# liruiluo/VLA-Adapter

Hardware: AMD Instinct MI355X
Metric: fine-tune samples/sec (224px img + 32-tok prompt), adapter-only, fwd+bwd+AdamW (higher is better)
Workload: dtype bf16

## Files before the change

vla_adapter_amd/csrc/gemm256.hip:

```cpp
#include <type_traits>
#include "gemm_epilogue.h"
#include "gemm_params.h"

namespace {

constexpr int BK = 64;
constexpr int HT = 16384;
constexpr int LDS_BYTES = 8 * HT;
constexpr int STG = 8192;

#define VLA_MMA_QUADRANT(Q, FB, FA)                                                                                                   \
  do {                                                                                                                                \
    if constexpr (F8) {                                                                                                               \
      _Pragma("unroll") for (int ni = 0; ni < 2; ++ni)                                                                                \
        _Pragma("unroll") for (int mi = 0; mi < 4; ++mi)                                                                              \
          Q[ni][mi] = __builtin_amdgcn_mfma_scale_f32_16x16x128_f8f6f4(cat8(FB[ni][0], FB[ni][1]), cat8(FA[mi][0], FA[mi][1]), Q[ni][mi], \
                                                                       0, 0, 0, 0x7f7f7f7f, 0, 0x7f7f7f7f);                            \
    } else {                                                                                                                          \
      _Pragma("unroll") for (int s = 0; s < 2; ++s)                                                                                   \
        _Pragma("unroll") for (int ni = 0; ni < 2; ++ni)                                                                              \
          _Pragma("unroll") for (int mi = 0; mi < 4; ++mi)                                                                            \
            Q[ni][mi] = __builtin_amdgcn_mfma_f32_16x16x32_bf16(FB[ni][s], FA[mi][s], Q[ni][mi], 0, 0, 0);                            \
    }                                                                                                                                 \
  } while (0)

template <int EPI, bool F8 = false, bool RES = true, bool R2 = false, bool EXT = false>
__global__ __launch_bounds__(512) void gemm256_kernel(GemmP p) {
  extern __shared__ __attribute__((aligned(16))) char smem[];
  constexpr int EB = F8 ? 1 : 2;
  constexpr bool HAS_RES = EPI == 0 && RES;
  constexpr bool PRE = EPI != 2;
  const int tid = threadIdx.x, lane = tid & 63;
  const int wid = __builtin_amdgcn_readfirstlane(tid >> 6);
  const int wr = wid >> 2, wc = wid & 3;

  const int G = gridDim.x, bid = blockIdx.x;
  const int total = p.ntiles * p.batch;
  const int q8 = total >> 3, r8 = total & 7;
  const int xcd = bid & 7;
  auto rstart = [&](int x) { return x < r8 ? x * (q8 + 1) : r8 * (q8 + 1) + (x - r8) * q8; };
  int vt = bid;
  constexpr int GM = 6;
  int m0, n0, z;
  const char* Ab; const char* Bb;
  unsigned oa[2][2], ob[2][2];
  unsigned oa2[EXT ? 2 : 1][2], ob2[EXT ? 2 : 1][2];
  auto setup = [&](int swz) {
    int sl = lane;
    asm volatile("" : "+v"(sl));
    const int kc = ((sl & 7) ^ ((sl >> 3) & 7)) * 16;
    const int lrow = sl >> 3;
    int gA = p.gA;
    asm volatile("" : "+s"(gA));
    int ntl = p.ntiles;
    asm volatile("" : "+s"(ntl));
    z = swz / ntl;
    const int tl = swz - z * ntl;
    int br = ntl / p.tiles_n, bc = p.tiles_n;
    asm volatile("" : "+s"(br), "+s"(bc));
    const int pgb = GM * bc;
    const int grp = tl / pgb, rem = tl - grp * pgb;
    const int gmr = min(GM, br - grp * GM);
    m0 = (grp * GM + rem % gmr) * 256;
    n0 = (rem / gmr) * 256;
    Ab = reinterpret_cast<const char*>(p.A) + (long long)z * p.sA * EB;
    Bb = reinterpret_cast<const char*>(p.B) + (long long)z * p.sB * EB;
#pragma unroll
    for (int h = 0; h < 2; ++h)
#pragma unroll
      for (int j = 0; j < 2; ++j) {
        const int ra = min(m0 + wr * 128 + h * 64 + (wid & 3) * 16 + j * 8 + lrow, p.M - 1);
        oa[h][j] = (unsigned)(grouped_row(ra, gA, p.sgA, p.lda) * EB + kc);
        const int rb = min(n0 + (wid >> 1) * 64 + h * 32 + (wid & 1) * 16 + j * 8 + lrow, p.N - 1);
        ob[h][j] = (unsigned)((long long)rb * p.ldb * EB + kc);
        if constexpr (EXT) {
          oa2[h][j] = (unsigned)((long long)ra * p.lda2 * 2 + kc);
          ob2[h][j] = (unsigned)((long long)rb * p.ldb2 * 2 + kc);
        }
      }
  };
  const unsigned wdst = (unsigned)(size_t)((__attribute__((address_space(3))) char*)smem) + wid * 2048;
  auto stage_a = [&](int slot, int h, int k0) {
    if (EXT && k0 >= p.K) {
      const char* b2 = reinterpret_cast<const char*>(p.A2) + (k0 - p.K) * 2;
      glds16s(b2, oa2[EXT ? h : 0][0], wdst + slot * HT);
      glds16s(b2, oa2[EXT ? h : 0][1], wdst + slot * HT + 1024);
      return;
    }
    glds16s(Ab + k0 * 2, oa[h][0], wdst + slot * HT);
    glds16s(Ab + k0 * 2, oa[h][1], wdst + slot * HT + 1024);
  };
  auto stage_b = [&](int slot, int h, int k0) {
    if (EXT && k0 >= p.K) {
      const char* b2 = reinterpret_cast<const char*>(p.B2) + (k0 - p.K) * 2;
      glds16s(b2, ob2[EXT ? h : 0][0], wdst + slot * HT);
      glds16s(b2, ob2[EXT ? h : 0][1], wdst + slot * HT + 1024);
      return;
    }
    glds16s(Bb + k0 * 2, ob[h][0], wdst + slot * HT);
    glds16s(Bb + k0 * 2, ob[h][1], wdst + slot * HT + 1024);
  };
  auto stage_k0 = [&](int buf) {
    stage_b(buf * 4 + 0, 0, 0); stage_a(buf * 4 + 1, 0, 0); stage_b(buf * 4 + 2, 1, 0); stage_a(buf * 4 + 3, 1, 0);
  };
  uint2 braw[4];
  auto bias_vec = [&]() {
    const bf16_t* bias = (EPI != 2 && p.bias) ? p.bias + (long long)z * p.sBias : nullptr;
    return bias != nullptr && (((size_t)bias & 7) == 0) && p.N >= 4;
  };
  auto fetch_bias = [&](bool bvec) {
    int sl = lane;
    asm volatile("" : "+v"(sl));
    const int lq = sl >> 4;
    long long dist = bvec ? (long long)((uintptr_t)(p.bias + (long long)z * p.sBias) - (uintptr_t)p.B) : 0;
    int lim = bvec ? p.N : 0;
    asm volatile("" : "+s"(dist), "+s"(lim));
    const bf16_t* src = reinterpret_cast<const bf16_t*>(reinterpret_cast<const char*>(p.B) + dist);
#pragma unroll
    for (int t4 = 0; t4 < 4; ++t4) {
      const int n = n0 + wc * 64 + t4 * 16 + lq * 4;
      braw[t4] = *reinterpret_cast<const uint2*>(src + (n + 3 < lim ? n : 0));
    }
  };

  const int nt = p.K / (F8 ? 2 * BK : BK) + (EXT ? p.K2 / BK : 0);

  const int aoff = wr * 64 * 128, boff = wc * 32 * 128;

  int cur = rstart(xcd) + (bid >> 3);
  if (p.stagger > 0 && (total - 1 - bid) / G + 1 < (total + G - 1) / G) {
    for (int i = 0; i < p.stagger; ++i) __builtin_amdgcn_s_sleep(16);
  }
  setup(cur);
  stage_k0(0);
  int d = 0;

  for (;;) {
    vt += G;
    const int nxt = vt < total ? rstart(vt & 7) + (vt >> 3) : -1;
    asm volatile("" : "+s"(cur));
    setup(cur);
    const bool bvec = bias_vec();
    if (nt > 1) {
      const int sn = (d ^ 1) * 4;
      stage_b(sn + 0, 0, BK); stage_a(sn + 1, 0, BK); stage_b(sn + 2, 1, BK);
    }
    fetch_bias(bvec);
    if (nt > 1) asm volatile("s_waitcnt vmcnt(10)" ::: "memory");
    else asm volatile("s_waitcnt vmcnt(4)" ::: "memory");
    VLA_BARRIER();
    int fl = lane;
    asm volatile("" : "+v"(fl));
    const int fo0 = (fl & 15) * 128 + ((((F8 ? 2 * (fl >> 4) : 0 + (fl >> 4))) ^ (fl & 7)) << 4);
    const int fo1 = (fl & 15) * 128 + ((((F8 ? 2 * (fl >> 4) + 1 : 4 + (fl >> 4))) ^ (fl & 7)) << 4);
    if (wr == 1) VLA_BARRIER();

    f32x4 acc[2][2][2][4];
#pragma unroll
    for (int a = 0; a < 2; ++a)
#pragma unroll
      for (int b = 0; b < 2; ++b)
#pragma unroll
        for (int c = 0; c < 2; ++c)
#pragma unroll
          for (int e = 0; e < 4; ++e) acc[a][b][c][e] = f32x4{0.f, 0.f, 0.f, 0.f};

    bf16x8 fa[4][2], fb0[2][2], fb1[2][2];
    for (int t = 0; t < nt; ++t) {
      const char* kb = smem + d * 4 * HT;
      const int so = d * 4, sn = (d ^ 1) * 4;
      {
        const char* sb = kb + 0 * HT + boff;
#pragma unroll
        for (int ni = 0; ni < 2; ++ni) {
          fb0[ni][0] = *reinterpret_cast<const bf16x8*>(sb + ni * 2048 + fo0);
          fb0[ni][1] = *reinterpret_cast<const bf16x8*>(sb + ni * 2048 + fo1);
        }
        const char* sa = kb + 1 * HT + aoff;
#pragma unroll
        for (int mi = 0; mi < 4; ++mi) {
          fa[mi][0] = *reinterpret_cast<const bf16x8*>(sa + mi * 2048 + fo0);
          fa[mi][1] = *reinterpret_cast<const bf16x8*>(sa + mi * 2048 + fo1);
        }
        const char* sb1 = kb + 2 * HT + boff;
#pragma unroll
        for (int ni = 0; ni < 2; ++ni) {
          fb1[ni][0] = *reinterpret_cast<const bf16x8*>(sb1 + ni * 2048 + fo0);
          fb1[ni][1] = *reinterpret_cast<const bf16x8*>(sb1 + ni * 2048 + fo1);
        }
        __builtin_amdgcn_sched_barrier(0);
        if (t + 1 < nt) {
          stage_a(sn + 3, 1, (t + 1) * BK);
          if (t > 0) asm volatile("s_waitcnt vmcnt(8)" ::: "memory");
        } else if (t > 0) {
          asm volatile("s_waitcnt vmcnt(0)" ::: "memory");
        }
        asm volatile("s_waitcnt lgkmcnt(0)" ::: "memory");
        VLA_BARRIER();
        __builtin_amdgcn_s_setprio(1);
        VLA_MMA_QUADRANT(acc[0][0], fb0, fa);
        VLA_MMA_QUADRANT(acc[0][1], fb1, fa);
        __builtin_amdgcn_s_setprio(0);
        VLA_BARRIER();
      }
      {
        const char* sa = kb + 3 * HT + aoff;
#pragma unroll
        for (int mi = 0; mi < 4; ++mi) {
          fa[mi][0] = *reinterpret_cast<const bf16x8*>(sa + mi * 2048 + fo0);
          fa[mi][1] = *reinterpret_cast<const bf16x8*>(sa + mi * 2048 + fo1);
        }
        __builtin_amdgcn_sched_barrier(0);
        if (t + 2 < nt) {
          stage_b(so + 0, 0, (t + 2) * BK); stage_a(so + 1, 0, (t + 2) * BK); stage_b(so + 2, 1, (t + 2) * BK);
          asm volatile("s_waitcnt vmcnt(8)" ::: "memory");
        } else if (t + 1 < nt) {
          asm volatile("s_waitcnt vmcnt(2)" ::: "memory");
        } else {
          asm volatile("s_waitcnt vmcnt(0)" ::: "memory");
        }
        asm volatile("s_waitcnt lgkmcnt(0)" ::: "memory");
        VLA_BARRIER();
        __builtin_amdgcn_s_setprio(1);
        VLA_MMA_QUADRANT(acc[1][1], fb1, fa);
        VLA_MMA_QUADRANT(acc[1][0], fb0, fa);
        __builtin_amdgcn_s_setprio(0);
        VLA_BARRIER();
      }
      d ^= 1;
    }
    if (wr == 0) VLA_BARRIER();
    asm volatile("s_waitcnt lgkmcnt(0)" ::: "memory");

    const int em0 = m0, en0 = n0, ez = z;
    int el = lane;
    asm volatile("" : "+v"(el));
    const int lq = el >> 4, lr = el & 15;
    int gR = p.gR, gC = p.gC, res_mod = p.res_mod, c_live_mod = p.c_live_mod;
    asm volatile("" : "+s"(gR), "+s"(gC), "+s"(res_mod), "+s"(c_live_mod));
    const bf16_t* bias = (EPI != 2 && p.bias) ? p.bias + (long long)ez * p.sBias : nullptr;
    const int wn0 = en0 + wc * 64;
    if constexpr (F8) {
#pragma unroll
      for (int t4 = 0; t4 < 4; ++t4) {
        float sbv[4];
#pragma unroll
        for (int j = 0; j < 4; ++j) sbv[j] = p.scaleB[min(wn0 + t4 * 16 + lq * 4 + j, p.N - 1)];
#pragma unroll
        for (int mh = 0; mh < 2; ++mh)
#pragma unroll
          for (int mi = 0; mi < 4; ++mi) {
            const float sav = p.scaleA[min(em0 + wr * 128 + mh * 64 + mi * 16 + lr, p.M - 1)];
#pragma unroll
            for (int j = 0; j < 4; ++j) acc[mh][t4 >> 1][t4 & 1][mi][j] *= sav * sbv[j];
          }
      }
    }
    float bv[4][4];
    int ebvec = __builtin_amdgcn_readfirstlane(bias_vec() ? 1 : 0);
    asm volatile("" : "+s"(ebvec));
#pragma unroll
    for (int t4 = 0; t4 < 4; ++t4) {
      const int n = wn0 + t4 * 16 + lq * 4;
      const bool ok = ebvec != 0 && n + 3 < p.N;
      bv[t4][0] = ok ? bf_lo(braw[t4].x) : 0.f; bv[t4][1] = ok ? bf_hi(braw[t4].x) : 0.f;
      bv[t4][2] = ok ? bf_lo(braw[t4].y) : 0.f; bv[t4][3] = ok ? bf_hi(braw[t4].y) : 0.f;
      if (bias && !ok) {
#pragma unroll
        for (int j = 0; j < 4; ++j)
          if (n + j < p.N) bv[t4][j] = bf2f(bias[n + j]);
      }
    }
    bf16_t* Cb = p.C + (long long)ez * p.sC;
    const bf16_t* Rb = (HAS_RES && p.R) ? p.R + (long long)ez * p.sR : nullptr;
    const bool vec_ok = ((p.ldc & 7) == 0) && (!Rb || (p.ldr & 7) == 0);
    const bool plain_rows = (res_mod | gR | gC | c_live_mod) == 0;
    const bool live_rows = EPI == 1 && (res_mod | gR | gC) == 0 && c_live_mod >= 64;
    bool skip[2], inside[2], fastm[2];
#pragma unroll
    for (int mh = 0; mh < 2; ++mh) {
      const int wm0 = em0 + wr * 128 + mh * 64;
      skip[mh] = wm0 >= p.M || wn0 >= p.N;
      inside[mh] = wm0 + 64 <= p.M && wn0 + 64 <= p.N;
      fastm[mh] = EPI != 2 && (plain_rows || live_rows) && vec_ok && inside[mh] && !skip[mh];
    }
    u32x4 rv[2][8];
    int fres0 = 0, fres1 = 0;
    const char* rsrc = nullptr;
    if constexpr (HAS_RES) {
      long long rdist = Rb ? (long long)((uintptr_t)Rb - (uintptr_t)p.B) : 0;
      fres0 = __builtin_amdgcn_readfirstlane((fastm[0] && Rb) ? 1 : 0);
      fres1 = __builtin_amdgcn_readfirstlane((fastm[1] && Rb) ? 1 : 0);
      asm volatile("" : "+s"(rdist), "+s"(fres0), "+s"(fres1));
      rsrc = reinterpret_cast<const char*>(p.B) + rdist;
    }
    auto load_res = [&](int mh, int it0, int it1) {
#pragma unroll
      for (int it = it0; it < it1; ++it) {
        const long long off = ((long long)(em0 + wr * 128 + mh * 64 + it * 8 + (el >> 3)) * p.ldr + wn0 + (el & 7) * 8) * 2;
        rv[mh][it] = *reinterpret_cast<const u32x4*>(rsrc + ((mh == 0 ? fres0 : fres1) ? off : 0));
      }
    };
    auto drop_res = [&](int mh) {
      asm volatile("" ::"v"(rv[mh][0]), "v"(rv[mh][1]), "v"(rv[mh][2]), "v"(rv[mh][3]), "v"(rv[mh][4]), "v"(rv[mh][5]), "v"(rv[mh][6]),
                   "v"(rv[mh][7]));
    };
    if (PRE && nxt >= 0) { setup(nxt); stage_k0(d); }
    char* const reg = PRE ? smem + (d ^ 1) * 4 * HT + wid * STG : smem + wid * STG;
    if constexpr (HAS_RES) load_res(0, 0, 4);

    if constexpr (EPI == 2) {
#pragma unroll
      for (int mh = 0; mh < 2; ++mh) {
        const int wm0 = em0 + wr * 128 + mh * 64;
        auto A4 = [&](int t4, int mi) -> f32x4& { return acc[mh][t4 >> 1][t4 & 1][mi]; };
          const bf16_t* GU = p.R + (long long)ez * p.sR;
          bf16_t* Cb = p.C + (long long)ez * p.sC;
          constexpr int ROWB = 2 * 64 * 2 + 16;
          char* reg2 = smem + wid * (32 * ROWB);
#pragma unroll
          for (int half = 0; half < 2; ++half) {
#pragma unroll
            for (int mq = 0; mq < 2; ++mq) {
              const int mi = 2 * half + mq;
              const int m = min(wm0 + mi * 16 + lr, p.M - 1);
#pragma unroll
              for (int t4 = 0; t4 < 4; ++t4) {
                const int hc = wn0 + t4 * 16 + lq * 4;
                const long long go = grouped_row(m, gR, p.sgR, p.ldr) + (hc >> 4) * 32 + (hc & 15);
                const bool ok = hc + 3 < p.N;
                const uint2 gv = ok ? *reinterpret_cast<const uint2*>(GU + go) : uint2{0, 0};
                const uint2 uv = ok ? *reinterpret_cast<const uint2*>(GU + go + 16) : uint2{0, 0};
                float gg[4], uu[4], dg[4], du[4];
                unpack4(gv, gg);
                unpack4(uv, uu);
#pragma unroll
                for (int j = 0; j < 4; ++j) swiglu_bwd(rbf(A4(t4, mi)[j] * p.alpha), gg[j], uu[j], dg[j], du[j]);
                char* rowp = reg2 + (mq * 16 + lr) * ROWB + (t4 * 32 + lq * 4) * 2;
                *reinterpret_cast<uint2*>(rowp) = pack4(dg);
                *reinterpret_cast<uint2*>(rowp + 32) = pack4(du);
              }
            }
#pragma unroll
            for (int it = 0; it < 8; ++it) {
              const int row = it * 4 + (el >> 4), ch = el & 15;
              const int m = wm0 + half * 32 + row, n2 = 2 * wn0 + ch * 8;
              if (m < p.M && n2 + 8 <= 2 * p.N)
                *reinterpret_cast<uint4*>(Cb + (long long)m * p.ldc + n2) = *reinterpret_cast<const uint4*>(reg2 + row * ROWB + ch * 16);
            }
          }
      }
    } else {
      uint2 pk[2][4][4];
      uint2 hp[2][2][4];
      if constexpr (EPI == 1) {
        const bool plain = bias == nullptr && p.alpha == 1.f;
#pragma unroll
        for (int mh = 0; mh < 2; ++mh)
#pragma unroll
          for (int pr = 0; pr < 2; ++pr)
#pragma unroll
            for (int mi = 0; mi < 4; ++mi) {
              f32x4 ga = acc[mh][pr][0][mi], ua = acc[mh][pr][1][mi];
              if (!plain) {
#pragma unroll
                for (int j = 0; j < 4; ++j) { ga[j] = epi_linear(ga[j], p.alpha, bv[2 * pr][j]); ua[j] = epi_linear(ua[j], p.alpha, bv[2 * pr + 1][j]); }
              }
              const uint2 gp = pack4(ga), up = pack4(ua);
              float g[4], u[4], h[4];
              unpack4(gp, g);
              unpack4(up, u);
#pragma unroll
              for (int j = 0; j < 4; ++j) h[j] = swiglu_h(g[j], u[j]);
              pk[mh][2 * pr][mi] = gp;
              pk[mh][2 * pr + 1][mi] = up;
              hp[mh][pr][mi] = pack4(h);
            }
      } else {
        auto phase_a = [&](auto fn, auto post_t) {
          constexpr bool POST = decltype(post_t)::value;
          const float alpha = p.alpha;
#pragma unroll
          for (int mh = 0; mh < 2; ++mh)
#pragma unroll
            for (int t4 = 0; t4 < 4; ++t4)
#pragma unroll
              for (int mi = 0; mi < 4; ++mi) {
                const f32x4 a = acc[mh][t4 >> 1][t4 & 1][mi];
                float x[4];
#pragma unroll
                for (int j = 0; j < 4; ++j) {
                  x[j] = fn(epi_linear<POST>(a[j], alpha, bv[t4][j]));
                }
                pk[mh][t4][mi] = uint2{pack2(x[0], x[1]), pack2(x[2], x[3])};
              }
        };
        auto phase_a_rope = [&]() {
          const float alpha = p.alpha;
#pragma unroll
          for (int mh = 0; mh < 2; ++mh)
#pragma unroll
            for (int mi = 0; mi < 4; ++mi) {
              const int pos = min(em0 + wr * 128 + mh * 64 + mi * 16 + lr, p.M - 1) % p.rope_T;
#pragma unroll
              for (int ni = 0; ni < 2; ++ni) {
                const int d = ni * 16 + lq * 4;
                const f32x4 c = *reinterpret_cast<const f32x4*>(p.rope_cos + (long long)pos * 32 + d);
                const f32x4 sn = *reinterpret_cast<const f32x4*>(p.rope_sin + (long long)pos * 32 + d);
                const f32x4 xa = acc[mh][0][ni][mi], xb = acc[mh][1][ni][mi];
                float ya[4], yb[4];
#pragma unroll
                for (int j = 0; j < 4; ++j) {
                  const float a = rbf(epi_linear(xa[j], alpha, bv[ni][j])), b = rbf(epi_linear(xb[j], alpha, bv[ni + 2][j]));
                  ya[j] = rope_rot_a(a, b, c[j], sn[j]);
                  yb[j] = rope_rot_b(a, b, c[j], sn[j]);
                }
                pk[mh][ni][mi] = uint2{pack2(ya[0], ya[1]), pack2(ya[2], ya[3])};
                pk[mh][ni + 2][mi] = uint2{pack2(yb[0], yb[1]), pack2(yb[2], yb[3])};
              }
              __builtin_amdgcn_sched_barrier(0);
            }
        };
        auto phase_a_rope2 = [&](auto post_t) {
          constexpr bool POST = decltype(post_t)::value;
          const float alpha = p.alpha;
#pragma unroll
          for (int mh = 0; mh < 2; ++mh)
#pragma unroll
            for (int mi = 0; mi < 4; ++mi) {
              const int pos = min(em0 + wr * 128 + mh * 64 + mi * 16 + lr, p.M - 1) % p.rope_T;
#pragma unroll
              for (int t4 = 0; t4 < 4; ++t4) {
                const int d = (wn0 + t4 * 16 + lq * 4) % p.rope_dh;
                const f32x4 c = *reinterpret_cast<const f32x4*>(p.rope_cos + (long long)pos * p.rope_dh + d);
                const f32x4 sn = *reinterpret_cast<const f32x4*>(p.rope_sin + (long long)pos * p.rope_dh + d);
                const f32x4 a = acc[mh][t4 >> 1][t4 & 1][mi];
                float x[4];
#pragma unroll
                for (int j = 0; j < 4; ++j) {
                  x[j] = rbf(epi_linear<POST>(a[j], alpha, bv[t4][j]));
                }
                const float y0 = rope_rot_a(x[0], x[1], c[0], sn[0]), y1 = rope_rot_b(x[0], x[1], c[1], sn[1]);
                const float y2 = rope_rot_a(x[2], x[3], c[2], sn[2]), y3 = rope_rot_b(x[2], x[3], c[3], sn[3]);
                pk[mh][t4][mi] = uint2{pack2(y0, y1), pack2(y2, y3)};
                if (t4 & 1) __builtin_amdgcn_sched_barrier(0);
              }
            }
        };
        if (p.rope_mode == 1 && wn0 < p.rope_cols) phase_a_rope();
        else if (R2 && p.rope_mode == 2 && wn0 < p.rope_cols) {
          if (p.bias_post) phase_a_rope2(std::true_type{});
          else phase_a_rope2(std::false_type{});
        } else if (p.bias_post) phase_a(ActNone{}, std::true_type{});
        else if (p.act == VLA_ACT_GELU) phase_a(ActGelu{}, std::false_type{});
        else if (p.act == VLA_ACT_RELU) phase_a(ActRelu{}, std::false_type{});
        else if (p.act == VLA_ACT_GELU_TANH) phase_a(ActGeluTanh{}, std::false_type{});
        else phase_a(ActNone{}, std::false_type{});
      }
#pragma unroll
      for (int mh = 0; mh < 2; ++mh)
#pragma unroll
        for (int t4 = 0; t4 < 4; ++t4)
          asm volatile("" : "+v"(pk[mh][t4][0].x), "+v"(pk[mh][t4][0].y), "+v"(pk[mh][t4][1].x), "+v"(pk[mh][t4][1].y),
                            "+v"(pk[mh][t4][2].x), "+v"(pk[mh][t4][2].y), "+v"(pk[mh][t4][3].x), "+v"(pk[mh][t4][3].y));
      asm volatile("" : "+v"(el));
      if constexpr (HAS_RES) { load_res(0, 4, 8); load_res(1, 0, 8); }
#pragma unroll
      for (int mh = 0; mh < 2; ++mh) {
        const int wm0 = em0 + wr * 128 + mh * 64;
        if (skip[mh]) {
          if constexpr (HAS_RES) drop_res(mh);
          continue;
        }
        if constexpr (EPI == 1) {
          bf16_t* C2 = p.C2 + (long long)ez * p.sC2;
          constexpr int HSTR = 32 * 2 + 16;
#pragma unroll
          for (int pr = 0; pr < 2; ++pr)
#pragma unroll
            for (int mi = 0; mi < 4; ++mi)
              *reinterpret_cast<uint2*>(reg + (mi * 16 + lr) * HSTR + (pr * 16 + lq * 4) * 2) = hp[mh][pr][mi];
          const bool hvec = ((p.ldc2 & 7) == 0) && (((size_t)C2 & 15) == 0);
          uint4 hv[4];
#pragma unroll
          for (int it = 0; it < 4; ++it) hv[it] = *reinterpret_cast<const uint4*>(reg + (it * 16 + (el >> 2)) * HSTR + (el & 3) * 16);
          __builtin_amdgcn_sched_barrier(0);
#pragma unroll
          for (int it = 0; it < 4; ++it) {
            const int row = it * 16 + (el >> 2), ch = el & 3;
            const int m = wm0 + row, hc = (wn0 >> 1) + ch * 8;
            const uint4 v = hv[it];
            if (hvec && inside[mh]) {
              *reinterpret_cast<uint4*>(C2 + (long long)m * p.ldc2 + hc) = v;
              continue;
            }
            if (m >= p.M || hc >= (p.N >> 1)) continue;
            bf16_t* dst = C2 + (long long)m * p.ldc2 + hc;
            if (hvec && hc + 8 <= (p.N >> 1)) {
              *reinterpret_cast<uint4*>(dst) = v;
            } else {
              const unsigned wv[4] = {v.x, v.y, v.z, v.w};
#pragma unroll
              for (int k = 0; k < 8; ++k)
                if (hc + k < (p.N >> 1)) dst[k] = (bf16_t)((k & 1) ? (wv[k >> 1] >> 16) : (wv[k >> 1] & 0xffffu));
            }
          }
          if (p.C == nullptr) continue;
          if (c_live_mod > 0 && (wm0 % c_live_mod) + 63 < p.c_live_from) continue;
        }
#pragma unroll
        for (int t4 = 0; t4 < 4; ++t4)
#pragma unroll
          for (int mi = 0; mi < 4; ++mi) {
            const int row = mi * 16 + lr;
            *reinterpret_cast<uint2*>(reg + row * 128 + (((t4 * 2 + (lq >> 1)) ^ ((row >> 1) & 7)) << 4) + (lq & 1) * 8) = pk[mh][t4][mi];
          }
        if (fastm[mh]) {
          uint4 vv[8];
#pragma unroll
          for (int it = 0; it < 8; ++it) {
            const int row = it * 8 + (el >> 3), ch = el & 7;
            vv[it] = *reinterpret_cast<const uint4*>(reg + row * 128 + ((ch ^ ((row >> 1) & 7)) << 4));
          }
          __builtin_amdgcn_sched_barrier(0);
          auto store_fast = [&](auto live_t) {
          constexpr bool LIVE = decltype(live_t)::value;
          int lpos = 0;
          if constexpr (LIVE) lpos = __builtin_amdgcn_readfirstlane(wm0 % c_live_mod);
#pragma unroll
          for (int it = 0; it < 8; ++it) {
            const int row = it * 8 + (el >> 3), ch = el & 7;
            if constexpr (LIVE) {
              int pos = lpos + row;
              if (pos >= c_live_mod) pos -= c_live_mod;
              if (pos < p.c_live_from) continue;
            }
            uint4 v = vv[it];
            if constexpr (HAS_RES) {
              const u32x4 r = rv[mh][it];
              const unsigned a[4] = {v.x, v.y, v.z, v.w};
              unsigned o[4];
#pragma unroll
              for (int k = 0; k < 4; ++k) o[k] = (mh == 0 ? fres0 : fres1) ? add_packed2(a[k], r[k]) : a[k];
              v = uint4{o[0], o[1], o[2], o[3]};
            }
            *reinterpret_cast<uint4*>(Cb + (long long)(wm0 + row) * p.ldc + wn0 + ch * 8) = v;
          }
          };
          if (EPI == 1 && c_live_mod > 0) store_fast(std::true_type{});
          else store_fast(std::false_type{});
          continue;
        }
        auto store_rows = [&](auto fast_t) {
          constexpr bool FAST = decltype(fast_t)::value;
#pragma nounroll
          for (int it = 0; it < 8; ++it) {
            const int row = it * 8 + (el >> 3), ch = el & 7;
            const int m = wm0 + row, n = wn0 + ch * 8;
            uint4 v = *reinterpret_cast<const uint4*>(reg + row * 128 + ((ch ^ ((row >> 1) & 7)) << 4));
            if (m >= p.M || n >= p.N) continue;
            long long roff, crow;
            if constexpr (FAST) {
              roff = (long long)m * p.ldr;
              crow = (long long)m * p.ldc;
            } else {
              if (!row_live(m, c_live_mod, p.c_live_from)) continue;
              roff = residual_row(m, res_mod, gR, p.sgR, p.ldr);
              crow = grouped_row(m, gC, p.sgC, p.ldc);
            }
            if (vec_ok && n + 8 <= p.N) {
              if (Rb) v = add_packed8(v, *reinterpret_cast<const uint4*>(Rb + roff + n));
              *reinterpret_cast<uint4*>(Cb + crow + n) = v;
            } else {
              store_tail8(Cb, crow, Rb, roff, v, n, p.N);
            }
          }
        };
        if constexpr (HAS_RES) drop_res(mh);
        if (plain_rows) store_rows(std::true_type{});
        else store_rows(std::false_type{});
      }
    }

    if (nxt < 0) break;
    VLA_BARRIER();
    if (!PRE) { setup(nxt); stage_k0(d); }
    cur = nxt;
  }
}

int num_cus() {
  static int n = 0;
  if (n == 0) {
    int dev = 0;
    if (hipGetDevice(&dev) != hipSuccess || hipDeviceGetAttribute(&n, hipDeviceAttributeMultiprocessorCount, dev) != hipSuccess || n <= 0) n = 256;
  }
  return n;
}

template <int EPI, bool F8 = false, bool RES = true, bool R2 = false, bool EXT = false>
int launch256(const GemmP& p0, int batch, long long grid, hipStream_t st) {
  if (int rc = vla_lds_limit<gemm256_kernel<EPI, F8, RES, R2, EXT>>(LDS_BYTES, "gemm256_kernel")) return rc;
  GemmP p = p0;
  p.tiles_n = (p.N + 255) / 256;
  p.ntiles = ((p.M + 255) / 256) * p.tiles_n;
  p.batch = batch;
  const long long total = (long long)p.ntiles * batch;
  if (grid <= 0 || grid > total) grid = total;
  p.stagger = 0;
  if (total > grid && total % grid != 0) {
    const long long tile_cycles = (long long)((p.K + (EXT ? p.K2 : 0)) / BK) * 2128 + 13000;
    p.stagger = (int)(tile_cycles / 2 / 1024);
  }
  hipLaunchKernelGGL((gemm256_kernel<EPI, F8, RES, R2, EXT>), dim3((unsigned)grid), dim3(512), LDS_BYTES, st, p);
  return VLA_OK;
}

}

int vla_num_cus() { return num_cus(); }

int vla_gemm256_launch(const GemmP& p, int epi, int batch, long long grid, hipStream_t st) {
  if (p.K2 > 0) {
    if (epi == 1) return launch256<1, false, true, false, true>(p, 1, grid, st);
    return p.R ? launch256<0, false, true, false, true>(p, 1, grid, st) : launch256<0, false, false, false, true>(p, 1, grid, st);
  }
  if (p.scaleA != nullptr) return epi == 1 ? launch256<1, true>(p, batch, grid, st) : launch256<0, true>(p, batch, grid, st);
  if (p.rope_mode == 2) return launch256<0, false, false, true>(p, batch, grid, st);
  if (epi == 1) return launch256<1>(p, batch, grid, st);
  if (epi == 2) return launch256<2>(p, batch, grid, st);
  return p.R ? launch256<0, false, true>(p, batch, grid, st) : launch256<0, false, false>(p, batch, grid, st);
}
```

vla_adapter_amd/csrc/gemm_epilogue.h:

```cpp
#pragma once
#include "common.h"
#include "../../include/vla_native.h"

template <bool POST = false>
__device__ __forceinline__ float epi_linear(float acc, float alpha, float bias) {
  return POST ? rbf(acc * alpha) + bias : acc * alpha + bias;
}

struct ActNone { __device__ __forceinline__ float operator()(float v) const { return v; } };
struct ActGelu { __device__ __forceinline__ float operator()(float v) const { return gelu_erf(rbf(v)); } };
struct ActRelu { __device__ __forceinline__ float operator()(float v) const { return fmaxf(v, 0.f); } };
struct ActGeluTanh { __device__ __forceinline__ float operator()(float v) const { return gelu_tanh(rbf(v)); } };
template <class Body>
__device__ __forceinline__ void epi_with_act(int act, Body&& body) {
  if (act == VLA_ACT_GELU) body(ActGelu{});
  else if (act == VLA_ACT_RELU) body(ActRelu{});
  else if (act == VLA_ACT_GELU_TANH) body(ActGeluTanh{});
  else body(ActNone{});
}

__device__ __forceinline__ float rope_rot_a(float a, float b, float c, float s) { return rbf(a * c) + rbf(-b * s); }
__device__ __forceinline__ float rope_rot_b(float a, float b, float c, float s) { return rbf(b * c) + rbf(a * s); }
template <int N, class X, class T>
__device__ __forceinline__ void rope_half(X& a, X& b, const T& c, const T& s) {
#pragma unroll
  for (int j = 0; j < N; ++j) {
    const float x = rbf(a[j]), y = rbf(b[j]);
    a[j] = rope_rot_a(x, y, c[j], s[j]);
    b[j] = rope_rot_b(x, y, c[j], s[j]);
  }
}

__device__ __forceinline__ float sigmoid_rcp(float g) { return __builtin_amdgcn_rcpf(1.0f + __expf(-g)); }
__device__ __forceinline__ float silu_grad(float g, float sg) { return sg * (1.0f + g * (1.0f - sg)); }
__device__ __forceinline__ float swiglu_h(float g, float u) { return rbf(g * sigmoid_rcp(g)) * u; }
__device__ __forceinline__ void swiglu_bwd(float d, float g, float u, float& dg, float& du) {
  const float sg = sigmoid_rcp(g);
  du = d * g * sg;
  dg = d * u * silu_grad(g, sg);
}

__device__ __forceinline__ unsigned add_packed2(unsigned a, unsigned r) { return pack2(bf_lo(a) + bf_lo(r), bf_hi(a) + bf_hi(r)); }
template <class R>
__device__ __forceinline__ uint4 add_packed8(const uint4& a, const R& r) {
  if constexpr (__is_same(R, uint4)) return uint4{add_packed2(a.x, r.x), add_packed2(a.y, r.y), add_packed2(a.z, r.z), add_packed2(a.w, r.w)};
  else return uint4{add_packed2(a.x, r[0]), add_packed2(a.y, r[1]), add_packed2(a.z, r[2]), add_packed2(a.w, r[3])};
}
__device__ __forceinline__ void add_residual4(float (&v)[4], const uint2& r) {
  float rr[4];
  unpack4(r, rr);
#pragma unroll
  for (int j = 0; j < 4; ++j) v[j] = rbf(v[j]) + rr[j];
}
__device__ __forceinline__ void store_tail8(bf16_t* c, long long crow, const bf16_t* r, long long roff, const uint4& v, int n, int N) {
  const unsigned wv[4] = {v.x, v.y, v.z, v.w};
#pragma unroll
  for (int k = 0; k < 8; ++k) {
    if (n + k < N) {
      float f = (k & 1) ? bf_hi(wv[k >> 1]) : bf_lo(wv[k >> 1]);
      if (r) f += bf2f(r[roff + n + k]);
      c[crow + n + k] = f2bf(f);
    }
  }
}

__device__ __forceinline__ long long grouped_row(int m, int g, long long stride, int ld) {
  return g > 0 ? (long long)(m / g) * stride + (long long)(m % g) * ld : (long long)m * ld;
}
__device__ __forceinline__ long long residual_row(int m, int res_mod, int g, long long stride, int ld) {
  return res_mod > 0 ? (long long)(m % res_mod) * ld : grouped_row(m, g, stride, ld);
}
__device__ __forceinline__ bool row_live(int m, int mod, int from) { return !(mod > 0 && (m % mod) < from); }
```

Before: 1321.

## Move RoPE into store phase with pipelined cos/sin fetches in 256-tile GEMM

Rotary embedding is no longer applied per accumulator fragment in registers. It now runs after the tile is staged through LDS, in the row-major store phase, where cos/sin loads are issued one batch ahead and overlap with LDS unstaging and global stores. Half-split (mode 1) RoPE without residual is also routed to the R2 kernel variant so it uses the same path. A slow per-row fallback handles partial tiles. The cost is a larger, more complex epilogue with higher register pressure and new layout-dependent index math.

```diff
diff --git a/vla_adapter_amd/csrc/gemm256.hip b/vla_adapter_amd/csrc/gemm256.hip
--- a/vla_adapter_amd/csrc/gemm256.hip
+++ b/vla_adapter_amd/csrc/gemm256.hip
@@ -421,37 +421,9 @@
               __builtin_amdgcn_sched_barrier(0);
             }
         };
-        auto phase_a_rope2 = [&](auto post_t) {
-          constexpr bool POST = decltype(post_t)::value;
-          const float alpha = p.alpha;
-#pragma unroll
-          for (int mh = 0; mh < 2; ++mh)
-#pragma unroll
-            for (int mi = 0; mi < 4; ++mi) {
-              const int pos = min(em0 + wr * 128 + mh * 64 + mi * 16 + lr, p.M - 1) % p.rope_T;
-#pragma unroll
-              for (int t4 = 0; t4 < 4; ++t4) {
-                const int d = (wn0 + t4 * 16 + lq * 4) % p.rope_dh;
-                const f32x4 c = *reinterpret_cast<const f32x4*>(p.rope_cos + (long long)pos * p.rope_dh + d);
-                const f32x4 sn = *reinterpret_cast<const f32x4*>(p.rope_sin + (long long)pos * p.rope_dh + d);
-                const f32x4 a = acc[mh][t4 >> 1][t4 & 1][mi];
-                float x[4];
-#pragma unroll
-                for (int j = 0; j < 4; ++j) {
-                  x[j] = rbf(epi_linear<POST>(a[j], alpha, bv[t4][j]));
-                }
-                const float y0 = rope_rot_a(x[0], x[1], c[0], sn[0]), y1 = rope_rot_b(x[0], x[1], c[1], sn[1]);
-                const float y2 = rope_rot_a(x[2], x[3], c[2], sn[2]), y3 = rope_rot_b(x[2], x[3], c[3], sn[3]);
-                pk[mh][t4][mi] = uint2{pack2(y0, y1), pack2(y2, y3)};
-                if (t4 & 1) __builtin_amdgcn_sched_barrier(0);
-              }
-            }
-        };
-        if (p.rope_mode == 1 && wn0 < p.rope_cols) phase_a_rope();
-        else if (R2 && p.rope_mode == 2 && wn0 < p.rope_cols) {
-          if (p.bias_post) phase_a_rope2(std::true_type{});
-          else phase_a_rope2(std::false_type{});
-        } else if (p.bias_post) phase_a(ActNone{}, std::true_type{});
+        if (!R2 && p.rope_mode == 1 && wn0 < p.rope_cols) phase_a_rope();
+        else if (p.bias_post) phase_a(ActNone{}, std::true_type{});
+        else if (R2 && p.rope_mode != 0 && wn0 < p.rope_cols) phase_a(ActNone{}, std::false_type{});
         else if (p.act == VLA_ACT_GELU) phase_a(ActGelu{}, std::false_type{});
         else if (p.act == VLA_ACT_RELU) phase_a(ActRelu{}, std::false_type{});
         else if (p.act == VLA_ACT_GELU_TANH) phase_a(ActGeluTanh{}, std::false_type{});
@@ -465,9 +437,157 @@
                             "+v"(pk[mh][t4][2].x), "+v"(pk[mh][t4][2].y), "+v"(pk[mh][t4][3].x), "+v"(pk[mh][t4][3].y));
       asm volatile("" : "+v"(el));
       if constexpr (HAS_RES) { load_res(0, 4, 8); load_res(1, 0, 8); }
+      int rmode = 0;
+      bool roped = false;
+      int rd0 = 0, rd1 = 0;
+      if constexpr (R2) {
+        rmode = wn0 < p.rope_cols ? p.rope_mode : 0;
+        rd0 = (wn0 + (el & 7) * 8) % p.rope_dh;
+        rd1 = rd0 + 4 >= p.rope_dh ? rd0 + 4 - p.rope_dh : rd0 + 4;
+        if (rmode != 0 && fastm[0] && fastm[1] && p.rope_T >= 64) {
+          roped = true;
+          const int rT = p.rope_T;
+          const int lp0 = __builtin_amdgcn_readfirstlane((em0 + wr * 128) % rT);
+          int lp1 = lp0 + 64;
+          if (lp1 >= rT) lp1 -= rT;
+          f32x4 ta[4][4], tb[4][4];
+          auto stage = [&](int mh) {
+#pragma unroll
+            for (int t4 = 0; t4 < 4; ++t4)
+#pragma unroll
+              for (int mi = 0; mi < 4; ++mi) {
+                const int row = mi * 16 + lr;
+                *reinterpret_cast<uint2*>(reg + row * 128 + (((t4 * 2 + (lq >> 1)) ^ ((row >> 1) & 7)) << 4) + (lq & 1) * 8) = pk[mh][t4][mi];
+              }
+          };
+          auto fetch = [&](f32x4 (&t)[4], unsigned o0, unsigned o1) {
+            t[0] = *reinterpret_cast<const f32x4*>(reinterpret_cast<const char*>(p.rope_cos) + o0);
+            t[1] = *reinterpret_cast<const f32x4*>(reinterpret_cast<const char*>(p.rope_cos) + o1);
+            t[2] = *reinterpret_cast<const f32x4*>(reinterpret_cast<const char*>(p.rope_sin) + o0);
+            t[3] = *reinterpret_cast<const f32x4*>(reinterpret_cast<const char*>(p.rope_sin) + o1);
+          };
+          if (rmode == 2) {
+            auto request = [&](f32x4 (&t)[4][4], int lp, int it0) {
+#pragma unroll
+              for (int k = 0; k < 4; ++k) {
+                int pos = lp + (it0 + k) * 8 + (el >> 3);
+                if (pos >= rT) pos -= rT;
+                fetch(t[k], (unsigned)(pos * p.rope_dh + rd0) * 4u, (unsigned)(pos * p.rope_dh + rd1) * 4u);
+              }
+            };
+            auto unstage = [&](uint4 (&vv)[4], int it0) {
+#pragma unroll
+              for (int k = 0; k < 4; ++k) {
+                const int row = (it0 + k) * 8 + (el >> 3), ch = el & 7;
+                vv[k] = *reinterpret_cast<const uint4*>(reg + row * 128 + ((ch ^ ((row >> 1) & 7)) << 4));
+              }
+            };
+            auto rotate_store = [&](const f32x4 (&t)[4][4], const uint4 (&vv)[4], int mh, int it0) {
+#pragma unroll
+              for (int k = 0; k < 4; ++k) {
+                const int row = (it0 + k) * 8 + (el >> 3), ch = el & 7;
+                *reinterpret_cast<uint4*>(Cb + (long long)(em0 + wr * 128 + mh * 64 + row) * p.ldc + wn0 + ch * 8) =
+                    rope_inter8(vv[k], t[k][0], t[k][1], t[k][2], t[k][3]);
+              }
+            };
+            uint4 va[4], vb[4];
+            request(ta, lp0, 0);
+            stage(0);
+            unstage(va, 0);
+            __builtin_amdgcn_sched_barrier(0);
+            request(tb, lp0, 4);
+            __builtin_amdgcn_sched_barrier(0);
+            rotate_store(ta, va, 0, 0);
+            unstage(vb, 4);
+            __builtin_amdgcn_sched_barrier(0);
+            request(ta, lp1, 0);
+            __builtin_amdgcn_sched_barrier(0);
+            rotate_store(tb, vb, 0, 4);
+            stage(1);
+            unstage(va, 0);
+            __builtin_amdgcn_sched_barrier(0);
+            request(tb, lp1, 4);
+            __builtin_amdgcn_sched_barrier(0);
+            rotate_store(ta, va, 1, 0);
+            unstage(vb, 4);
+            rotate_store(tb, vb, 1, 4);
+          } else {
+            auto request = [&](f32x4 (&t)[4][4], int lp, int k0) {
+#pragma unroll
+              for (int k = 0; k < 2; ++k) {
+                int pos = lp + (k0 + k) * 16 + (el >> 2);
+                if (pos >= rT) pos -= rT;
+                const unsigned o = (unsigned)(pos * 32 + (el & 3) * 8) * 4u;
+                fetch(t[k], o, o + 16u);
+              }
+            };
+            auto unstage = [&](uint4 (&vl)[2], uint4 (&vh)[2], int k0) {
+#pragma unroll
+              for (int k = 0; k < 2; ++k) {
+                const int row = (k0 + k) * 16 + (el >> 2), c = el & 3;
+                vl[k] = *reinterpret_cast<const uint4*>(reg + row * 128 + ((c ^ ((row >> 1) & 7)) << 4));
+                vh[k] = *reinterpret_cast<const uint4*>(reg + row * 128 + (((c + 4) ^ ((row >> 1) & 7)) << 4));
+              }
+            };
+            auto rotate_store = [&](const f32x4 (&t)[4][4], uint4 (&vl)[2], uint4 (&vh)[2], int mh, int k0) {
+#pragma unroll
+              for (int k = 0; k < 2; ++k) {
+                const int row = (k0 + k) * 16 + (el >> 2), c = el & 3;
+                rope_half8(vl[k], vh[k], t[k][0], t[k][1], t[k][2], t[k][3]);
+                bf16_t* dst = Cb + (long long)(em0 + wr * 128 + mh * 64 + row) * p.ldc + wn0 + c * 8;
+                *reinterpret_cast<uint4*>(dst) = vl[k];
+                *reinterpret_cast<uint4*>(dst + 32) = vh[k];
+              }
+            };
+            uint4 vl[2], vh[2];
+            request(ta, lp0, 0);
+            stage(0);
+            unstage(vl, vh, 0);
+            __builtin_amdgcn_sched_barrier(0);
+            request(tb, lp0, 2);
+            __builtin_amdgcn_sched_barrier(0);
+            rotate_store(ta, vl, vh, 0, 0);
+            unstage(vl, vh, 2);
+            __builtin_amdgcn_sched_barrier(0);
+            request(ta, lp1, 0);
+            __builtin_amdgcn_sched_barrier(0);
+            rotate_store(tb, vl, vh, 0, 2);
+            stage(1);
+            unstage(vl, vh, 0);
+            __builtin_amdgcn_sched_barrier(0);
+            request(tb, lp1, 2);
+            __builtin_amdgcn_sched_barrier(0);
+            rotate_store(ta, vl, vh, 1, 0);
+            unstage(vl, vh, 2);
+            rotate_store(tb, vl, vh, 1, 2);
+          }
+        }
+      }
+      auto rope_rows = [&](uint4& v, int m, int row, int ch) {
+        if constexpr (R2) {
+          const char* rc = reinterpret_cast<const char*>(p.rope_cos);
+          const char* rs = reinterpret_cast<const char*>(p.rope_sin);
+          const int pos = m % p.rope_T;
+          if (rmode == 2) {
+            const unsigned o0 = (unsigned)(pos * p.rope_dh + rd0) * 4u, o1 = (unsigned)(pos * p.rope_dh + rd1) * 4u;
+            v = rope_inter8(v, *reinterpret_cast<const f32x4*>(rc + o0), *reinterpret_cast<const f32x4*>(rc + o1),
+                            *reinterpret_cast<const f32x4*>(rs + o0), *reinterpret_cast<const f32x4*>(rs + o1));
+          } else if (rmode == 1) {
+            const uint4 pv = *reinterpret_cast<const uint4*>(reg + row * 128 + (((ch ^ 4) ^ ((row >> 1) & 7)) << 4));
+            const unsigned o = (unsigned)(pos * 32 + (ch & 3) * 8) * 4u;
+            const bool first = ch < 4;
+            uint4 lo{first ? v.x : pv.x, first ? v.y : pv.y, first ? v.z : pv.z, first ? v.w : pv.w};
+            uint4 hi{first ? pv.x : v.x, first ? pv.y : v.y, first ? pv.z : v.z, first ? pv.w : v.w};
+            rope_half8(lo, hi, *reinterpret_cast<const f32x4*>(rc + o), *reinterpret_cast<const f32x4*>(rc + o + 16),
+                       *reinterpret_cast<const f32x4*>(rs + o), *reinterpret_cast<const f32x4*>(rs + o + 16));
+            v = uint4{first ? lo.x : hi.x, first ? lo.y : hi.y, first ? lo.z : hi.z, first ? lo.w : hi.w};
+          }
+        }
+      };
 #pragma unroll
       for (int mh = 0; mh < 2; ++mh) {
         const int wm0 = em0 + wr * 128 + mh * 64;
+        if (R2 && roped) continue;
         if (skip[mh]) {
           if constexpr (HAS_RES) drop_res(mh);
           continue;
@@ -515,7 +635,7 @@
             const int row = mi * 16 + lr;
             *reinterpret_cast<uint2*>(reg + row * 128 + (((t4 * 2 + (lq >> 1)) ^ ((row >> 1) & 7)) << 4) + (lq & 1) * 8) = pk[mh][t4][mi];
           }
-        if (fastm[mh]) {
+        if (fastm[mh] && !(R2 && rmode != 0)) {
           uint4 vv[8];
 #pragma unroll
           for (int it = 0; it < 8; ++it) {
@@ -568,6 +688,7 @@
               roff = residual_row(m, res_mod, gR, p.sgR, p.ldr);
               crow = grouped_row(m, gC, p.sgC, p.ldc);
             }
+            rope_rows(v, m, row, ch);
             if (vec_ok && n + 8 <= p.N) {
               if (Rb) v = add_packed8(v, *reinterpret_cast<const uint4*>(Rb + roff + n));
               *reinterpret_cast<uint4*>(Cb + crow + n) = v;
@@ -626,7 +747,7 @@
     return p.R ? launch256<0, false, true, false, true>(p, 1, grid, st) : launch256<0, false, false, false, true>(p, 1, grid, st);
   }
   if (p.scaleA != nullptr) return epi == 1 ? launch256<1, true>(p, batch, grid, st) : launch256<0, true>(p, batch, grid, st);
-  if (p.rope_mode == 2) return launch256<0, false, false, true>(p, batch, grid, st);
+  if (p.rope_mode == 2 || (p.rope_mode == 1 && epi == 0 && !p.R)) return launch256<0, false, false, true>(p, batch, grid, st);
   if (epi == 1) return launch256<1>(p, batch, grid, st);
   if (epi == 2) return launch256<2>(p, batch, grid, st);
   return p.R ? launch256<0, false, true>(p, batch, grid, st) : launch256<0, false, false>(p, batch, grid, st);
diff --git a/vla_adapter_amd/csrc/gemm_epilogue.h b/vla_adapter_amd/csrc/gemm_epilogue.h
--- a/vla_adapter_amd/csrc/gemm_epilogue.h
+++ b/vla_adapter_amd/csrc/gemm_epilogue.h
@@ -29,6 +29,29 @@
     a[j] = rope_rot_a(x, y, c[j], s[j]);
     b[j] = rope_rot_b(x, y, c[j], s[j]);
   }
+}
+template <class T>
+__device__ __forceinline__ void rope_half8(uint4& a, uint4& b, const T& c0, const T& c1, const T& s0, const T& s1) {
+  float x[8], y[8], ya[8], yb[8];
+  unpack8(a, x);
+  unpack8(b, y);
+#pragma unroll
+  for (int j = 0; j < 8; ++j) {
+    const float c = j < 4 ? c0[j & 3] : c1[j & 3], s = j < 4 ? s0[j & 3] : s1[j & 3];
+    ya[j] = rope_rot_a(x[j], y[j], c, s);
+    yb[j] = rope_rot_b(x[j], y[j], c, s);
+  }
+  a = pack8(ya);
+  b = pack8(yb);
+}
+template <class T>
+__device__ __forceinline__ unsigned rope_inter_pair(unsigned w, const T& c, const T& s, int j) {
+  const float x0 = bf_lo(w), x1 = bf_hi(w);
+  return pack2(rope_rot_a(x0, x1, c[j], s[j]), rope_rot_b(x0, x1, c[j + 1], s[j + 1]));
+}
+template <class T>
+__device__ __forceinline__ uint4 rope_inter8(const uint4& v, const T& c0, const T& c1, const T& s0, const T& s1) {
+  return uint4{rope_inter_pair(v.x, c0, s0, 0), rope_inter_pair(v.y, c0, s0, 2), rope_inter_pair(v.z, c1, s1, 0), rope_inter_pair(v.w, c1, s1, 2)};
 }
 
 __device__ __forceinline__ float sigmoid_rcp(float g) { return __builtin_amdgcn_rcpf(1.0f + __expf(-g)); }
```

Result: no change. 1330 (median of 6 runs) (+0.7%).
